# ExistentialRobotics/CORSAIR

Measured on AMD Instinct MI355X. Metric: end-to-end queries/sec (embed+retrieve+register), Scan2CAD chair, higher is better.
Workload: dtype f32 sparse conv + embedding / f64 RANSAC, k-NN, Chamfer, top-k / f16 MFMA bounds and shortlists (survivors recounted in f64)

## Files before the change

corsair_amd/csrc/ransac.h:

```cpp
#pragma once
#include "common.h"

namespace cs {

struct RansacProb {
  int64_t off;
  int32_t m;
  int32_t est_k;
  int32_t best_cnt;
  int32_t best_itr;
  unsigned long long best_err;
  int32_t done;
  int32_t iters;
  int32_t n_cand;
  int32_t chunk_max;
  double best_T[12];
};

__device__ __forceinline__ RansacProb prob_view(const RansacProb* probs, int p) {
  RansacProb v = {};
  v.off = probs[p].off;
  v.m = probs[p].m;
  v.est_k = __atomic_load_n(&probs[p].est_k, __ATOMIC_RELAXED);
  v.done = __atomic_load_n(&probs[p].done, __ATOMIC_RELAXED);
  return v;
}

constexpr int XCD_SLOTS = 64;
struct XcdTab {
  int32_t v[8 * XCD_SLOTS];
};
__device__ __forceinline__ int xcd_problem(const int32_t* __restrict__ xcd_ptr, const XcdTab& tab, int i) {
  return xcd_ptr ? xcd_ptr[i] : tab.v[i];
}

constexpr int BMAX = 16384;
constexpr int RC_CHUNK = 256;
constexpr int RC_HYP = 256;
constexpr int PF_K = 16;
constexpr int PF_PITCH = 40;
constexpr int PF_PITCH1 = 24;
__host__ __device__ constexpr int pf_pitch(int nm) { return nm == 2 ? PF_PITCH : PF_PITCH1; }
constexpr int PF_ROWS = 192;
constexpr int PF_NG = 2;
constexpr int PF_HYP = 4 * 32 * PF_NG;
constexpr int PF_STAT = 17;
constexpr float PF_SMAX = 128.0f;
constexpr int PF_S2_CAP = 1024;
constexpr double PF_TCAP = 0.75;
constexpr int FEW_MAX = 1024;

__host__ __device__ static inline int64_t pf_padded(int64_t m) { return (m + PF_ROWS - 1) / PF_ROWS * PF_ROWS; }

struct Stage2Rows {
  const _Float16* A16;
  const float* c_h;
  const unsigned* stat;
  double tcap;
  _Float16* A16s;
  float* c_hs;
  int32_t* cnt2;
};

__device__ __forceinline__ double residual2_f64(const double (&R)[12], double sx, double sy, double sz,
                                                double qx, double qy, double qz) {
  const double dx = fma(R[2], sz, fma(R[1], sy, fma(R[0], sx, R[3]))) - qx;
  const double dy = fma(R[6], sz, fma(R[5], sy, fma(R[4], sx, R[7]))) - qy;
  const double dz = fma(R[10], sz, fma(R[9], sy, fma(R[8], sx, R[11]))) - qz;
  return fma(dz, dz, fma(dy, dy, dx * dx));
}

__device__ __forceinline__ _Float16 f16_of(double v) { return (_Float16)(float)v; }

__device__ __forceinline__ void pf_centre(const double* __restrict__ sums, int p, double (&mu)[6]) {
#pragma unroll
  for (int c = 0; c < 6; ++c) mu[c] = sums[p * 6 + c];
}

__device__ __forceinline__ void pf_emit_row(const RansacProb& pr, int p, int h, int bmax, const double (&R)[3][3], double (&t)[3],
                                            const unsigned* __restrict__ stat, const double* __restrict__ sums, double thr2,
                                            double tcap, _Float16* __restrict__ A16, float* __restrict__ c_h) {
  {
    double mu[6];
    pf_centre(sums, p, mu);
#pragma unroll
    for (int a = 0; a < 3; ++a) t[a] = t[a] + (R[a][0] * mu[0] + R[a][1] * mu[1] + R[a][2] * mu[2]) - mu[3 + a];
  }
  const double smax = (double)__uint_as_float(stat[p * PF_STAT]);
  const double tt = t[0] * t[0] + t[1] * t[1] + t[2] * t[2];
  const double tn = sqrt(tt);
  double a[16];
  a[0] = 1.0;
#pragma unroll
  for (int b = 0; b < 3; ++b) a[1 + b] = 2.0 * (R[0][b] * t[0] + R[1][b] * t[1] + R[2][b] * t[2]);
#pragma unroll
  for (int x = 0; x < 3; ++x)
#pragma unroll
    for (int b = 0; b < 3; ++b) a[4 + 3 * x + b] = -2.0 * R[x][b];
#pragma unroll
  for (int x = 0; x < 3; ++x) a[13 + x] = -2.0 * t[x];
  double dev = 0.0;
#pragma unroll
  for (int x = 0; x < 3; ++x)
#pragma unroll
    for (int y = 0; y < 3; ++y) {
      const double e = R[0][x] * R[0][y] + R[1][x] * R[1][y] + R[2][x] * R[2][y] - (x == y ? 1.0 : 0.0);
      dev = fmax(dev, fabs(e));
    }
  bool usable = smax <= (double)PF_SMAX && tn <= 4.0 * (double)PF_SMAX && dev < 1.0e-3;
  if (tcap > 0.0) usable = usable && tn <= tcap * smax;
  usable = usable && thr2 < 3.0e4;
  const double beta = tcap > 0.0 ? smax * smax : 0.0;
#pragma unroll
  for (int k = 0; k < 16; ++k) usable = usable && fabs(a[k]) < 6.0e4;
  union {
    _Float16 h[PF_K];
    uint4 v[2];
  } row;
  double drop = 0.0;
#pragma unroll
  for (int k = 0; k < 16; ++k) {
    const _Float16 hi = usable ? f16_of(a[k]) : (_Float16)0.0f;
    row.h[k] = hi;
    if (usable) drop += fabs(a[k] - (double)hi) * (double)__uint_as_float(stat[p * PF_STAT + 1 + k]);
  }
  uint4* dst = reinterpret_cast<uint4*>(A16 + ((int64_t)p * bmax + h) * PF_K);
  dst[0] = row.v[0];
  dst[1] = row.v[1];
  const double w = 2.0 * smax + tn;
  const double eps = 2.5e-5 * w * w + 6.0e-6 + 3.0 * dev * smax * smax + 1.000001 * drop;
  c_h[(int64_t)p * bmax + h] = usable ? __double2float_rd((tt + beta) - (thr2 + eps)) : -1.0f;
}

struct RansacIn {
  RansacProb* probs;
  int n_prob, m_max;
  int64_t tot1;
  float* pk;
  float4* pair32;
};
struct Front {
  int it0 = 0, b = 0, par = 0;
  bool pf = false, on_side = false;
  XcdTab xtab;
  const int32_t* xcd_prob = nullptr;
  int pslots = 1;
};

void ransac_launch_pack(const RansacIn& in, const float* src, const float* tgt, hipStream_t s);
void ransac_launch_hyp(const RansacIn& in, const Front& f, int ransac_n, uint64_t seed, int force_jacobi, double* hyp,
                       const unsigned* pf_stat, const double* pf_sums, double thr2, double tcap, _Float16* A16, float* c_h,
                       int32_t* cnt_zero, hipStream_t s);
void ransac_launch_images(const RansacIn& in, const int64_t* off16, const float* src, const float* tgt, double* sums,
                          unsigned* stat, unsigned long long* chk_stats, _Float16* B32, _Float16* B16, double tcap,
                          hipStream_t s);
unsigned ransac_launch_prefilter(int nm, const RansacIn& in, const int64_t* off16, const _Float16* B, const _Float16* A16,
                                 const float* c_h, const Front& f, int tiles, int splits, int32_t* cnt_up,
                                 unsigned long long* trace, const int32_t* n_list, hipStream_t s);
void ransac_launch_survivors(const RansacIn& in, const Front& f, const int32_t* cnt_up, int32_t* res_cnt,
                             unsigned long long* err_by_h, int32_t* hlist, int32_t* n_surv, const Stage2Rows& s2, hipStream_t s);
void ransac_launch_check(const RansacIn& in, const Front& f, const int32_t* exact, const int32_t* cnt_up, const int32_t* hlist,
                         const int32_t* n_surv, const int32_t* cnt2, unsigned long long* stats, hipStream_t s);
void ransac_launch_count_chunk(const RansacIn& in, const double* hyp, int it0, int b, int hpw, int tiles, int splits,
                               double thr2, int32_t* res_cnt, hipStream_t s);
void ransac_launch_count_list(const RansacIn& in, const double* hyp, int it0, int b, double thr2, int32_t* res_cnt,
                              const int32_t* hlist, const int32_t* n_surv, hipStream_t s);
void ransac_launch_count_few(const RansacIn& in, const double* hyp, double thr2, double scale, int32_t* res_cnt,
                             unsigned long long* err_by_h, const int32_t* hlist, const int32_t* n_surv, int fslots,
                             const int32_t* cnt2, hipStream_t s);
void ransac_launch_err(const RansacIn& in, const double* hyp, const int32_t* cand, double thr2, double scale,
                       unsigned long long* cand_err, hipStream_t s);

}
```

corsair_amd/csrc/ransac.hip:

```cpp
#include <math.h>

#include <algorithm>
#include <atomic>
#include <vector>

#include "ransac.h"

namespace cs {

__device__ __forceinline__ int est_bound(int c, int m, int ransac_n, double log_1mc, int est_k0) {
  const double ratio = fmin(1.0, (double)c / (double)m);
  double pw = 1.0;
  for (int j = 0; j < ransac_n; ++j) pw = pw * ratio;
  const double den = log(1.0 - pw);
  if (den < 0.0) {
    const double est = log_1mc / den;
    if (est < (double)est_k0) return (int)ceil(est);
  }
  return est_k0;
}

__global__ __launch_bounds__(256) void k_ransac_scan1(RansacProb* probs, int n_prob,
                                                     const int32_t* __restrict__ res_cnt, int it0,
                                                     int bcount, int bmax, int ransac_n,
                                                     int max_iter, double log_1mc,
                                                     int32_t* __restrict__ cand, int* n_active,
                                                     const unsigned long long* __restrict__ err_by_h,
                                                     const double* __restrict__ hyp, int32_t* __restrict__ next_nsurv,
                                                     int* __restrict__ next_nactive) {
  extern __shared__ int32_t lcnt[];
  const int p = blockIdx.x;
  if (err_by_h && threadIdx.x == 0) {
    next_nsurv[p] = 0;
    if (p == 0) *next_nactive = 0;
  }
  RansacProb pr = probs[p];
  if (pr.done) return;
  const int seg = (bcount + 63) / 64;
  {
    const int32_t* g = res_cnt + (int64_t)p * bmax;
    for (int h = threadIdx.x; h < bcount; h += 256) lcnt[h + h / seg] = g[h];
  }
  __syncthreads();
  if (threadIdx.x >= 64) return;
  const int lane = threadIdx.x;
  const int32_t* cnt = lcnt + lane;
  const int s0 = lane * seg, s1 = min(bcount, s0 + seg);
  int lmax = 0;
  for (int h = s0; h < s1; ++h)
    if (it0 + h < pr.est_k) lmax = max(lmax, cnt[h]);
  int incl = lmax;
#pragma unroll
  for (int off = 1; off < 64; off <<= 1) {
    const int o = __shfl_up(incl, off);
    if (lane >= off) incl = max(incl, o);
  }
  int pre = __shfl_up(incl, 1);
  if (lane == 0) pre = 0;
  pre = max(pre, pr.best_cnt);
  int stop = 0x7fffffff;
  {
    int cur = pre;
    int ek = cur > pr.best_cnt ? est_bound(cur, pr.m, ransac_n, log_1mc, pr.est_k) : pr.est_k;
    for (int h = s0; h < s1; ++h) {
      if (it0 + h >= ek) {
        stop = h;
        break;
      }
      const int c = cnt[h];
      if (c > cur) {
        cur = c;
        ek = est_bound(cur, pr.m, ransac_n, log_1mc, pr.est_k);
      }
    }
  }
#pragma unroll
  for (int off = 32; off >= 1; off >>= 1) stop = min(stop, __shfl_xor(stop, off));
  if (stop > bcount) stop = bcount;
  int cmax = 0;
  for (int h = s0; h < min(s1, stop); ++h) cmax = max(cmax, cnt[h]);
#pragma unroll
  for (int off = 32; off >= 1; off >>= 1) cmax = max(cmax, __shfl_xor(cmax, off));
  int new_ek = pr.est_k;
  if (cmax > pr.best_cnt) new_ek = est_bound(cmax, pr.m, ransac_n, log_1mc, pr.est_k);
  int ncand = 0;
  unsigned long long e_min = ~0ULL;
  int h_min = 0x7fffffff;
  if (cmax > 0 && cmax >= pr.best_cnt) {
    if (err_by_h) {
      for (int h = s0; h < min(s1, stop); ++h)
        if (cnt[h] == cmax) {
          const unsigned long long e = err_by_h[(int64_t)p * bmax + h];
          if (e < e_min) {
            e_min = e;
            h_min = h;
          }
        }
#pragma unroll
      for (int off = 32; off >= 1; off >>= 1) {
        const unsigned long long eo = __shfl_xor(e_min, off);
        const int ho = __shfl_xor(h_min, off);
        if (eo < e_min || (eo == e_min && ho < h_min)) {
          e_min = eo;
          h_min = ho;
        }
      }
    } else {
      int mine = 0;
      for (int h = s0; h < min(s1, stop); ++h) mine += cnt[h] == cmax;
      int incl2 = mine;
#pragma unroll
      for (int off = 1; off < 64; off <<= 1) {
        const int o = __shfl_up(incl2, off);
        if (lane >= off) incl2 += o;
      }
      int pos = incl2 - mine;
      ncand = __shfl(incl2, 63);
      for (int h = s0; h < min(s1, stop); ++h)
        if (cnt[h] == cmax) cand[(int64_t)p * bmax + pos++] = h;
    }
  }
  if (lane == 0) {
    const int consumed = it0 + stop;
    pr.est_k = new_ek;
    pr.n_cand = ncand;
    pr.chunk_max = cmax;
    if (consumed >= pr.est_k || consumed >= max_iter) {
      pr.done = 1;
      pr.iters = consumed < max_iter ? consumed : max_iter;
    } else {
      atomicAdd(n_active, 1);
    }
    if (err_by_h && h_min != 0x7fffffff && (cmax > pr.best_cnt || e_min < pr.best_err)) {
      pr.best_cnt = cmax;
      pr.best_err = e_min;
      pr.best_itr = it0 + h_min;
      for (int c = 0; c < 12; ++c) pr.best_T[c] = hyp[((int64_t)p * 12 + c) * bmax + h_min];
    }
    probs[p] = pr;
  }
}

__global__ void k_ransac_scan2(RansacProb* probs, int n_prob, const double* __restrict__ hyp,
                               const int32_t* __restrict__ cand,
                               const unsigned long long* __restrict__ cand_err, int by_h, int it0,
                               int bmax, int32_t* __restrict__ next_nsurv, int* __restrict__ next_nactive) {
  const int p = blockIdx.x * blockDim.x + threadIdx.x;
  if (p >= n_prob) return;
  next_nsurv[p] = 0;
  if (p == 0) *next_nactive = 0;
  RansacProb pr = probs[p];
  if (pr.n_cand <= 0) return;
  bool changed = false;
  int best_h = -1;
  for (int c = 0; c < pr.n_cand; ++c) {
    const unsigned long long e = cand_err[(int64_t)p * bmax + (by_h ? cand[(int64_t)p * bmax + c] : c)];
    if (pr.chunk_max > pr.best_cnt || e < pr.best_err) {
      pr.best_cnt = pr.chunk_max;
      pr.best_err = e;
      best_h = cand[(int64_t)p * bmax + c];
      changed = true;
    }
  }
  pr.n_cand = 0;
  if (changed) {
    pr.best_itr = it0 + best_h;
    for (int c = 0; c < 12; ++c) pr.best_T[c] = hyp[((int64_t)p * 12 + c) * bmax + best_h];
  }
  probs[p] = pr;
}

__global__ void k_ransac_finish(const RansacProb* __restrict__ probs, int n_prob, double scale,
                                float* __restrict__ T, int32_t* __restrict__ inliers,
                                double* __restrict__ rmse, int32_t* __restrict__ iters) {
  const int p = blockIdx.x * blockDim.x + threadIdx.x;
  if (p >= n_prob) return;
  const RansacProb pr = probs[p];
  float* o = T + (int64_t)p * 16;
  if (pr.best_cnt > 0) {
    for (int c = 0; c < 12; ++c) o[c] = (float)pr.best_T[c];
  } else {
    for (int c = 0; c < 12; ++c) o[c] = (c % 5 == 0) ? 1.f : 0.f;
  }
  o[12] = 0.f;
  o[13] = 0.f;
  o[14] = 0.f;
  o[15] = 1.f;
  if (inliers) inliers[p] = pr.best_cnt;
  if (rmse)
    rmse[p] = pr.best_cnt > 0 ? sqrt(((double)pr.best_err / scale) / (double)pr.best_cnt) : 0.0;
  if (iters) iters[p] = pr.iters;
}

}

using namespace cs;

namespace {
std::atomic<unsigned long long> g_pf_stats[5];

struct PinnedScratch {
  char* p = nullptr;
  size_t n = 0;
  ~PinnedScratch() {
    if (p) (void)hipHostFree(p);
  }
};
thread_local PinnedScratch t_pinned;
char* pinned_scratch(size_t bytes) {
  if (t_pinned.n < bytes) {
    if (t_pinned.p) (void)hipHostFree(t_pinned.p);
    t_pinned.p = nullptr;
    t_pinned.n = 0;
    void* q = nullptr;
    if (hipHostMalloc(&q, bytes, hipHostMallocDefault) != hipSuccess) return nullptr;
    t_pinned.p = static_cast<char*>(q);
    t_pinned.n = bytes;
  }
  return t_pinned.p;
}

struct Options {
  bool prefilter;
  bool check;
  int pf_nm;
  bool stage2;
  int first_chunk;
  int force_jacobi;
  bool overlap;
  int trace_it0;
  const char* trace_file;
};
Options read_options() {
  const char* pf = getenv("CS_RANSAC_PREFILTER");
  const char* ck = getenv("CS_RANSAC_CHECK");
  const char* k = getenv("CS_RANSAC_PF_K");
  const char* s2 = getenv("CS_RANSAC_STAGE2");
  const char* first = getenv("CS_RANSAC_FIRST");
  const char* jac = getenv("CS_RANSAC_JACOBI");
  const char* ov = getenv("CS_RANSAC_OVERLAP");
  const char* tr = getenv("CS_PF_TRACE");
  const char* trf = getenv("CS_PF_TRACE_FILE");
  Options o;
  o.prefilter = !(pf && pf[0] == '0');
  o.check = ck && ck[0] == '1';
  o.pf_nm = (k && atoi(k) == 32) ? 2 : 1;
  o.stage2 = !(s2 && s2[0] == '0');
  o.first_chunk = ((std::min(std::max(first ? atoi(first) : 64, 64), BMAX) + 63) / 64) * 64;
  o.force_jacobi = jac && atoi(jac) != 0;
  o.overlap = !(ov && ov[0] == '0');
  o.trace_it0 = tr ? atoi(tr) : -1;
  o.trace_file = trf ? trf : "/tmp/pf_trace.bin";
  return o;
}

struct Scratch {
  int n_prob = 0;
  size_t st_probs = 0, st_surv = 0, st_cnt = 0, st_bytes = 0;
  PoolBuf<char> state;
  char* h_state = nullptr;
  PoolBuf<float> pk;
  PoolBuf<float4> pair32;
  PoolBuf<double> hyp;
  PoolBuf<int32_t> res_cnt, cand;
  PoolBuf<unsigned long long> cand_err;
  PoolBuf<int64_t> off16;
  PoolBuf<_Float16> B16, A16;
  PoolBuf<float> c_h;
  PoolBuf<int32_t> cnt_up, hlist;
  PoolBuf<unsigned> pf_stat;
  PoolBuf<double> pf_sums;
  PoolBuf<_Float16> B32, A16s;
  PoolBuf<float> c_hs;
  PoolBuf<int32_t> cnt2;
  PoolBuf<int32_t> exact_dbg;
  PoolBuf<unsigned long long> chk_stats;
  PoolBuf<int32_t> xcd_buf;
  PoolBuf<unsigned long long> trace;
  size_t trace_cap = 1;

  bool alloc(int n, int64_t tot1, int64_t rows16, int pf_nm, bool pf, bool stage2, bool check, bool tracing) {
    n_prob = n;
    st_probs = sizeof(RansacProb) * (size_t)n;
    st_surv = ((sizeof(int32_t) * (size_t)n + 7) / 8) * 8;
    st_cnt = st_surv + 8;
    st_bytes = st_probs + 2 * st_cnt;
    h_state = pinned_scratch(st_bytes);
    const size_t nb = (size_t)n * BMAX, ns2 = (size_t)n * PF_S2_CAP;
    if (tracing) trace_cap = (size_t)8 * n * 64 * 16 * 16;
    return h_state && state.alloc(st_bytes) && pk.alloc((size_t)tot1 * 6) && pair32.alloc((size_t)tot1 * 2) &&
           hyp.alloc(2 * nb * 12) && res_cnt.alloc(nb) && cand.alloc(nb) && cand_err.alloc(nb) && off16.alloc(n + 1) &&
           B16.alloc(pf ? (size_t)rows16 * pf_pitch(pf_nm) : 8) && A16.alloc(pf ? 2 * nb * PF_K : 8) &&
           c_h.alloc(pf ? 2 * nb : 1) && cnt_up.alloc(pf ? 2 * nb : 1) && hlist.alloc(pf ? nb : 1) &&
           pf_stat.alloc((size_t)n * PF_STAT) && pf_sums.alloc((size_t)n * 6) &&
           B32.alloc(stage2 ? (size_t)rows16 * PF_PITCH : 8) && A16s.alloc(stage2 ? ns2 * PF_K : 8) &&
           c_hs.alloc(stage2 ? ns2 : 1) && cnt2.alloc(stage2 ? ns2 : 1) &&
           exact_dbg.alloc(check ? nb : 1) && chk_stats.alloc(4) && xcd_buf.alloc((size_t)16 * n) && trace.alloc(trace_cap);
  }
  RansacProb* probs() const { return reinterpret_cast<RansacProb*>(state.p); }
  int32_t* nsurv(int par) const { return reinterpret_cast<int32_t*>(state.p + st_probs + par * st_cnt); }
  int* nactive(int par) const { return reinterpret_cast<int*>(state.p + st_probs + par * st_cnt + st_surv); }
  const int32_t* h_nsurv(int par) const { return reinterpret_cast<const int32_t*>(h_state + st_probs + par * st_cnt); }
  int h_nactive(int par) const { return *reinterpret_cast<const int*>(h_state + st_probs + par * st_cnt + st_surv); }
  double* hyp_of(int par) const { return hyp.p + (size_t)par * n_prob * 12 * BMAX; }
  _Float16* A16_of(int par) const { return A16.p + (size_t)par * n_prob * BMAX * PF_K; }
  float* c_h_of(int par) const { return c_h.p + (size_t)par * n_prob * BMAX; }
  int32_t* cnt_up_of(int par) const { return cnt_up.p + (size_t)par * n_prob * BMAX; }
  int32_t* xcd_of(int par) const { return xcd_buf.p + (size_t)par * 8 * n_prob; }
};

struct Event {
  hipEvent_t e = nullptr;
  ~Event() {
    if (e) (void)hipEventDestroy(e);
  }
};
struct SideDrain {
  hipStream_t st = nullptr;
  bool clean = false;
  ~SideDrain() {
    if (st && !clean) (void)hipStreamSynchronize(st);
  }
};

struct RansacCall {
  int n_prob = 0, ransac_n = 0, max_iter = 0, m_max = 0;
  uint64_t seed = 0;
  int64_t total = 0, tot1 = 1;
  double thr2 = 0.0, scale = 0.0, log_1mc = 0.0, tcap = 0.0;
  Options opt;
  bool pf_alloc = false, stage2 = false, check = false;
  std::vector<RansacProb> hp;
  std::vector<int64_t> h_off16;
  std::vector<int32_t> h_xcd[2];
  Scratch sc;
  Event round_done, front_done[2], hyp_done[2];
  hipStream_t s = nullptr, side = nullptr, side_hyp = nullptr;
  SideDrain side_drain, side_hyp_drain;
  int max_surv_prev = 1 << 30;
  unsigned long long tot_surv = 0, tot_eval = 0;
  size_t trace_n = 0;

  int init(const int64_t* h_off, int n, double max_corr, int rn, int iters, double confidence, uint64_t sd, hipStream_t st);
  int setup(const float* d_src, const float* d_tgt);
  int open_streams();
  RansacIn in() const { return RansacIn{sc.probs(), n_prob, m_max, tot1, sc.pk.p, sc.pair32.p}; }
  bool prefiltered(int it0) const { return pf_alloc && it0 >= opt.first_chunk; }
  int chunk_of(int it0) const {
    const int b = it0 < opt.first_chunk ? opt.first_chunk : it0 < 512 ? 512 - it0 : (it0 < BMAX ? it0 : BMAX);
    return b > max_iter - it0 ? max_iter - it0 : b;
  }
  int chunk_splits(int tiles) const {
    int splits = (int)(4096 / ((int64_t)n_prob * tiles > 0 ? (int64_t)n_prob * tiles : 1));
    if (splits < 1) splits = 1;
    if (splits > 16) splits = 16;
    while (splits > 1 && m_max / splits < 4 * RC_CHUNK) --splits;
    return splits;
  }
  int place(int it0, int par, int* live);
  Front enqueue_front(int it0, int par, hipStream_t st);
  int back_half(const Front& cur);
  int count_chunk(const Front& cur, double eval_pairs);
  int count_survivors(const Front& cur, bool* err_known);
  bool read_back(const Front& cur);
  int finish(float* d_T, int32_t* d_inliers, double* d_rmse, int32_t* d_iters);
};

int RansacCall::init(const int64_t* h_off, int n, double max_corr, int rn, int iters, double confidence, uint64_t sd,
                     hipStream_t st) {
  n_prob = n;
  ransac_n = rn;
  max_iter = iters;
  seed = sd;
  s = st;
  total = h_off[n_prob] - h_off[0];
  tot1 = total ? total : 1;
  hp.resize(n_prob);
  h_off16.assign(n_prob + 1, 0);
  for (int p = 0; p < n_prob; ++p) {
    int64_t m = h_off[p + 1] - h_off[p];
    CS_REQUIRE(m >= 0 && m < (1LL << 24), CS_ERR_INVALID,
               "cs_ransac_batch: bad segment %d (a problem holds fewer than 2^24 correspondences)", p);
    RansacProb& pr = hp[p];
    memset(&pr, 0, sizeof(pr));
    pr.off = h_off[p];
    pr.m = (int32_t)m;
    pr.est_k = max_iter;
    pr.best_itr = -1;
    pr.done = m < ransac_n ? 1 : 0;
    if (m > m_max) m_max = (int)m;
    h_off16[p + 1] = h_off16[p] + pf_padded(m);
  }
  thr2 = max_corr * max_corr;
  int ex = 0;
  (void)frexp(thr2, &ex);
  scale = ldexp(1.0, 38 - ex);
  log_1mc = log(1.0 - confidence);
  opt = read_options();
  pf_alloc = opt.prefilter && total > 0 && max_iter > opt.first_chunk;
  stage2 = pf_alloc && opt.pf_nm == 1 && opt.stage2;
  check = pf_alloc && opt.check;
  tcap = opt.pf_nm == 2 ? 0.0 : PF_TCAP;
  const bool ok = sc.alloc(n_prob, tot1, h_off16[n_prob] ? h_off16[n_prob] : 1, opt.pf_nm, pf_alloc, stage2, check,
                           opt.trace_it0 >= 0);
  CS_REQUIRE(ok, CS_ERR_HIP, "cs_ransac_batch: scratch allocation failed");
  return CS_OK;
}

int RansacCall::setup(const float* d_src, const float* d_tgt) {
  memset(sc.h_state, 0, sc.st_bytes);
  memcpy(sc.h_state, hp.data(), sc.st_probs);
  CS_HIP_CHECK(hipMemcpyAsync(sc.state.p, sc.h_state, sc.st_bytes, hipMemcpyHostToDevice, s));
  if (pf_alloc) {
    CS_HIP_CHECK(hipMemcpyAsync(sc.off16.p, h_off16.data(), sizeof(int64_t) * (n_prob + 1),
                                hipMemcpyHostToDevice, s));
    ransac_launch_images(in(), sc.off16.p, d_src, d_tgt, sc.pf_sums.p, sc.pf_stat.p, sc.chk_stats.p,
                         opt.pf_nm == 2 ? sc.B16.p : (stage2 ? sc.B32.p : nullptr), opt.pf_nm == 1 ? sc.B16.p : nullptr, tcap, s);
    CS_LAUNCH_CHECK();
  } else if (total > 0) {
    ransac_launch_pack(in(), d_src, d_tgt, s);
    CS_LAUNCH_CHECK();
  }
  if (opt.trace_it0 >= 0) CS_HIP_CHECK(hipMemsetAsync(sc.trace.p, 0, sizeof(unsigned long long) * sc.trace_cap, s));
  return CS_OK;
}

int RansacCall::open_streams() {
  for (Event* ev : {&round_done, &front_done[0], &front_done[1], &hyp_done[0], &hyp_done[1]})
    CS_HIP_CHECK(hipEventCreateWithFlags(&ev->e, hipEventDisableTiming));
  side = opt.overlap ? side_stream() : nullptr;
  side_hyp = side ? side_stream(1) : nullptr;
  side_drain.st = side;
  side_hyp_drain.st = side_hyp;
  return CS_OK;
}

int RansacCall::place(int it0, int par, int* live) {
  std::vector<int> order;
  for (int p = 0; p < n_prob; ++p)
    if (!hp[p].done && hp[p].est_k > it0) order.push_back(p);
  *live = (int)order.size();
  std::sort(order.begin(), order.end(), [&](int a, int c) { return hp[a].m > hp[c].m; });
  std::vector<std::vector<int>> lists(8);
  int64_t load[8] = {0, 0, 0, 0, 0, 0, 0, 0};
  for (int p : order) {
    int best = 0;
    for (int x = 1; x < 8; ++x)
      if (load[x] < load[best]) best = x;
    lists[best].push_back(p);
    load[best] += pf_padded(hp[p].m);
  }
  int pslots = 1;
  for (int x = 0; x < 8; ++x) pslots = std::max(pslots, (int)lists[x].size());
  std::vector<int32_t>& tab = h_xcd[par];
  tab.assign((size_t)8 * pslots, -1);
  for (int x = 0; x < 8; ++x)
    for (size_t i = 0; i < lists[x].size(); ++i) tab[(size_t)x * pslots + i] = lists[x][i];
  return pslots;
}

Front RansacCall::enqueue_front(int it0, int par, hipStream_t st) {
  Front f;
  f.it0 = it0;
  f.b = chunk_of(it0);
  f.par = par;
  f.pf = prefiltered(it0);
  f.on_side = st != s;
  const int b = f.b;
  int live = 0;
  f.pslots = place(it0, par, &live);
  const int pslots = f.pslots;
  hipStream_t sh = (f.on_side && f.pf && side_hyp) ? side_hyp : st;
  if (pslots <= XCD_SLOTS) {
    memcpy(f.xtab.v, h_xcd[par].data(), sizeof(int32_t) * 8 * pslots);
  } else {
    (void)hipMemcpyAsync(sc.xcd_of(par), h_xcd[par].data(), sizeof(int32_t) * 8 * pslots, hipMemcpyHostToDevice, sh);
    f.xcd_prob = sc.xcd_of(par);
  }
  _Float16* A16_r = f.pf ? sc.A16_of(par) : nullptr;
  float* c_h_r = f.pf ? sc.c_h_of(par) : nullptr;
  int32_t* cnt_up_r = f.pf ? sc.cnt_up_of(par) : nullptr;
  const int ptiles = (b + PF_HYP - 1) / PF_HYP;
  int psplits = (int)((8 * 1024 + (int64_t)live * ptiles - 1) / std::max<int64_t>((int64_t)live * ptiles, 1));
  if (psplits < 1) psplits = 1;
  if (psplits > 16) psplits = 16;
  while (psplits > 1 && m_max / psplits < 8 * PF_ROWS) --psplits;
  {
    ProfScope prof("ransac_hyp", sh);
    int32_t* fz = psplits > 1 ? cnt_up_r : nullptr;
    ransac_launch_hyp(in(), f, ransac_n, seed, opt.force_jacobi, sc.hyp_of(par), sc.pf_stat.p, sc.pf_sums.p, thr2, tcap, A16_r,
                      c_h_r, fz, sh);
  }
  if (f.pf) {
    if (sh != st) {
      (void)hipEventRecord(hyp_done[par].e, sh);
      (void)hipStreamWaitEvent(st, hyp_done[par].e, 0);
    }
    ProfScope prof("ransac_pre", st);
    unsigned long long* tr = (opt.trace_it0 == it0) ? sc.trace.p : nullptr;
    const unsigned nblk = ransac_launch_prefilter(opt.pf_nm, in(), sc.off16.p, sc.B16.p, A16_r, c_h_r, f, ptiles, psplits,
                                                  cnt_up_r, tr, nullptr, st);
    if (tr) trace_n = (size_t)nblk * 16;
  }
  if (f.on_side) (void)hipEventRecord(front_done[par].e, st);
  return f;
}

int RansacCall::count_chunk(const Front& cur, double eval_pairs) {
  const int b = cur.b;
  const int hpw = b <= 64 ? 64 : RC_HYP;
  const int tiles = (b + hpw - 1) / hpw;
  const int splits = chunk_splits(tiles);
  if (splits > 1 || hpw != RC_HYP)
    CS_HIP_CHECK(hipMemset2DAsync(sc.res_cnt.p, sizeof(int32_t) * BMAX, 0, sizeof(int32_t) * b, n_prob, s));
  ProfScope prof("ransac_eval", s, 30.0 * eval_pairs);
  ransac_launch_count_chunk(in(), sc.hyp_of(cur.par), cur.it0, b, hpw, tiles, splits, thr2, sc.res_cnt.p, s);
  return CS_OK;
}

int RansacCall::count_survivors(const Front& cur, bool* err_known) {
  const int b = cur.b;
  const double* hyp_r = sc.hyp_of(cur.par);
  const int32_t* cnt_up_r = sc.cnt_up_of(cur.par);
  int32_t* const d_nsurv = sc.nsurv(cur.par);
  const int surv_cap = std::min(max_surv_prev, b);
  const bool few = max_surv_prev <= FEW_MAX || b <= FEW_MAX;
  const bool run_s2 = stage2 && few && surv_cap <= PF_S2_CAP;
  Stage2Rows s2rows{};
  if (run_s2) {
    s2rows.A16 = sc.A16_of(cur.par);
    s2rows.c_h = sc.c_h_of(cur.par);
    s2rows.stat = sc.pf_stat.p;
    s2rows.tcap = tcap;
    s2rows.A16s = sc.A16s.p;
    s2rows.c_hs = sc.c_hs.p;
    s2rows.cnt2 = sc.cnt2.p;
  }
  ransac_launch_survivors(in(), cur, cnt_up_r, sc.res_cnt.p, sc.cand_err.p, sc.hlist.p, d_nsurv, s2rows, s);
  {
    ProfScope prof("ransac_eval", s);
    if (few) {
      if (run_s2) {
        const int s2tiles = std::max(1, (std::min(b, PF_S2_CAP) + PF_HYP - 1) / PF_HYP);
        int s2splits = 8;
        while (s2splits > 1 && m_max / s2splits < 8 * PF_ROWS) --s2splits;
        ransac_launch_prefilter(2, in(), sc.off16.p, sc.B32.p, sc.A16s.p, sc.c_hs.p, cur, s2tiles, s2splits, sc.cnt2.p, nullptr,
                                d_nsurv, s);
      }
      const int fslots = surv_cap <= 256 ? 4 : 8;
      ransac_launch_count_few(in(), hyp_r, thr2, scale, sc.res_cnt.p, sc.cand_err.p, sc.hlist.p, d_nsurv, fslots,
                              run_s2 ? sc.cnt2.p : nullptr, s);
      *err_known = true;
    } else {
      ransac_launch_count_list(in(), hyp_r, cur.it0, b, thr2, sc.res_cnt.p, sc.hlist.p, d_nsurv, s);
    }
  }
  if (check) {
    const int tiles = (b + RC_HYP - 1) / RC_HYP;
    const int splits = chunk_splits(tiles);
    CS_HIP_CHECK(hipMemset2DAsync(sc.exact_dbg.p, sizeof(int32_t) * BMAX, 0, sizeof(int32_t) * b, n_prob, s));
    ransac_launch_count_chunk(in(), hyp_r, cur.it0, b, RC_HYP, tiles, splits, thr2, sc.exact_dbg.p, s);
    ransac_launch_check(in(), cur, sc.exact_dbg.p, cnt_up_r, sc.hlist.p, d_nsurv, run_s2 ? sc.cnt2.p : nullptr, sc.chk_stats.p, s);
  }
  return CS_OK;
}

int RansacCall::back_half(const Front& cur) {
  const int it0 = cur.it0, b = cur.b;
  double eval_pairs = 0.0;
  for (int p = 0; p < n_prob; ++p) {
    if (hp[p].done) continue;
    const int nh = std::min(hp[p].est_k - it0, b);
    if (nh > 0) {
      eval_pairs += (double)nh * (double)hp[p].m;
      tot_eval += (unsigned long long)nh;
    }
  }
  bool err_known = false;
  if (!cur.pf) {
    if (int rc = count_chunk(cur, eval_pairs)) return rc;
  } else {
    prof_add_units("ransac_pre", 30.0 * eval_pairs);
    if (int rc = count_survivors(cur, &err_known)) return rc;
  }
  static const hipError_t scan1_lds = hipFuncSetAttribute(
      reinterpret_cast<const void*>(k_ransac_scan1), hipFuncAttributeMaxDynamicSharedMemorySize, 80 * 1024);
  CS_REQUIRE(scan1_lds == hipSuccess, CS_ERR_HIP, "cs_ransac_batch: cannot reserve LDS for k_ransac_scan1");
  RansacProb* const d_probs = sc.probs();
  const double* hyp_r = sc.hyp_of(cur.par);
  int32_t* const next_nsurv = sc.nsurv(cur.par ^ 1);
  int* const next_nactive = sc.nactive(cur.par ^ 1);
  hipLaunchKernelGGL(k_ransac_scan1, dim3((unsigned)n_prob), dim3(256), sizeof(int32_t) * (b + 64), s, d_probs, n_prob,
                     sc.res_cnt.p, it0, b, BMAX, ransac_n, max_iter, log_1mc, sc.cand.p, sc.nactive(cur.par),
                     err_known ? sc.cand_err.p : (const unsigned long long*)nullptr, hyp_r, next_nsurv, next_nactive);
  if (!err_known) {
    ransac_launch_err(in(), hyp_r, sc.cand.p, thr2, scale, sc.cand_err.p, s);
    hipLaunchKernelGGL(k_ransac_scan2, dim3((unsigned)ceil_div(n_prob, 64)), dim3(64), 0, s,
                       d_probs, n_prob, hyp_r, sc.cand.p, sc.cand_err.p, 0, it0, BMAX, next_nsurv, next_nactive);
  }
  CS_LAUNCH_CHECK();
  return CS_OK;
}

bool RansacCall::read_back(const Front& cur) {
  if (cur.pf) {
    const int32_t* h_surv = sc.h_nsurv(cur.par);
    max_surv_prev = 0;
    for (int p = 0; p < n_prob; ++p)
      if (!hp[p].done) {
        tot_surv += (unsigned long long)h_surv[p];
        if (h_surv[p] > max_surv_prev) max_surv_prev = h_surv[p];
      }
  }
  memcpy(hp.data(), sc.h_state, sc.st_probs);
  return sc.h_nactive(cur.par) != 0;
}

int RansacCall::finish(float* d_T, int32_t* d_inliers, double* d_rmse, int32_t* d_iters) {
  if (trace_n) {
    std::vector<unsigned long long> ht(trace_n);
    CS_HIP_CHECK(hipMemcpy(ht.data(), sc.trace.p, sizeof(unsigned long long) * trace_n, hipMemcpyDeviceToHost));
    FILE* f = fopen(opt.trace_file, "wb");
    if (f) {
      fwrite(ht.data(), sizeof(unsigned long long), trace_n, f);
      fclose(f);
    }
  }
  g_pf_stats[3] += tot_surv;
  g_pf_stats[4] += tot_eval;
  if (check) {
    unsigned long long h_stats[4] = {0, 0, 0, 0};
    CS_HIP_CHECK(hipMemcpyAsync(h_stats, sc.chk_stats.p, sizeof(h_stats), hipMemcpyDeviceToHost, s));
    CS_HIP_CHECK(hipStreamSynchronize(s));
    g_pf_stats[0] += h_stats[0];
    g_pf_stats[1] += h_stats[1];
    g_pf_stats[2] += h_stats[2];
    CS_REQUIRE(h_stats[0] == 0, CS_ERR_INTERNAL,
               "cs_ransac_batch: prefilter bound violated for %llu hypotheses", h_stats[0]);
  }
  hipLaunchKernelGGL(k_ransac_finish, dim3((unsigned)ceil_div(n_prob, 64)), dim3(64), 0, s,
                     sc.probs(), n_prob, scale, d_T, d_inliers, d_rmse, d_iters);
  CS_LAUNCH_CHECK();
  CS_HIP_CHECK(hipStreamSynchronize(s));
  side_drain.clean = true;
  side_hyp_drain.clean = true;
  return CS_OK;
}
}

extern "C" {

void cs_ransac_prefilter_stats(uint64_t out[5], int reset) {
  for (int i = 0; i < 5; ++i) {
    if (out) out[i] = g_pf_stats[i].load();
    if (reset) g_pf_stats[i].store(0);
  }
}

int cs_ransac_batch(const float* d_src, const float* d_tgt, const int64_t* h_off, int n_prob,
                    double max_corr, int ransac_n, int max_iter, double confidence, uint64_t seed,
                    float* d_T, int32_t* d_inliers, double* d_rmse, int32_t* d_iters,
                    void* stream) {
  CS_REQUIRE(h_off && d_T, CS_ERR_INVALID, "cs_ransac_batch: NULL argument");
  CS_REQUIRE(ransac_n >= 3 && ransac_n <= 64, CS_ERR_INVALID,
             "cs_ransac_batch: ransac_n %d not in [3, 64]", ransac_n);
  CS_REQUIRE(max_corr > 0.0 && max_iter >= 1, CS_ERR_INVALID,
             "cs_ransac_batch: need max_corr > 0 and max_iter >= 1");
  CS_REQUIRE(confidence > 0.0 && confidence <= 1.0, CS_ERR_INVALID,
             "cs_ransac_batch: confidence must be in (0, 1]");
  if (n_prob <= 0) return CS_OK;
  hipStream_t s = (hipStream_t)stream;
  pool_use_stream(s);
  const int64_t total = h_off[n_prob] - h_off[0];
  CS_REQUIRE(h_off[0] == 0 && total >= 0, CS_ERR_INVALID, "cs_ransac_batch: bad offsets");
  CS_REQUIRE(total == 0 || (d_src && d_tgt), CS_ERR_INVALID, "cs_ransac_batch: NULL correspondences");
  RansacCall c;
  if (int rc = c.init(h_off, n_prob, max_corr, ransac_n, max_iter, confidence, seed, s)) return rc;
  if (int rc = c.setup(d_src, d_tgt)) return rc;
  if (int rc = c.open_streams()) return rc;

  Front cur = c.enqueue_front(0, 0, s);
  CS_LAUNCH_CHECK();
  bool side_pending = false;
  int side_par = 0;
  while (true) {
    if (cur.on_side) {
      CS_HIP_CHECK(hipStreamWaitEvent(s, c.front_done[cur.par].e, 0));
      side_pending = false;
    }
    if (int rc = c.back_half(cur)) return rc;
    CS_HIP_CHECK(hipMemcpyAsync(c.sc.h_state, c.sc.state.p, c.sc.st_bytes, hipMemcpyDeviceToHost, s));
    CS_HIP_CHECK(hipEventRecord(c.round_done.e, s));
    Front nxt;
    const int it1 = cur.it0 + cur.b;
    const bool have_next = it1 < max_iter;
    if (have_next) {
      nxt = c.enqueue_front(it1, cur.par ^ 1, (c.side && cur.pf && c.prefiltered(it1)) ? c.side : s);
      if (nxt.on_side) {
        side_pending = true;
        side_par = nxt.par;
      }
      CS_LAUNCH_CHECK();
    }
    CS_HIP_CHECK(hipEventSynchronize(c.round_done.e));
    const bool active = c.read_back(cur);
    if (!active || !have_next) break;
    cur = nxt;
  }
  if (side_pending) CS_HIP_CHECK(hipStreamWaitEvent(s, c.front_done[side_par].e, 0));
  return c.finish(d_T, d_inliers, d_rmse, d_iters);
}

}
```

corsair_amd/csrc/ransac_hyp.hip:

```cpp
#include "ransac.h"
#include "exact_div.h"
#include "horn.h"

namespace cs {


__global__ void k_ransac_pack(const float* __restrict__ src, const float* __restrict__ tgt,
                              int64_t n, float* __restrict__ pk, float4* __restrict__ pair32) {
  int64_t i = blockIdx.x * (int64_t)blockDim.x + threadIdx.x;
  if (i >= n) return;
  pair32[2 * i + 0] = make_float4(src[3 * i + 0], src[3 * i + 1], src[3 * i + 2], tgt[3 * i + 0]);
  pair32[2 * i + 1] = make_float4(tgt[3 * i + 1], tgt[3 * i + 2], 0.f, 0.f);
  pk[0 * n + i] = src[3 * i + 0];
  pk[1 * n + i] = src[3 * i + 1];
  pk[2 * n + i] = src[3 * i + 2];
  pk[3 * n + i] = tgt[3 * i + 0];
  pk[4 * n + i] = tgt[3 * i + 1];
  pk[5 * n + i] = tgt[3 * i + 2];
}

__device__ __forceinline__ void centroid_div(double (&cs_)[3], double (&ct_)[3], double dn, double inv_n) {
  bool fast = inv_n != 0.0;
#pragma unroll
  for (int a = 0; a < 3; ++a) fast = fast && exact_div_ok(cs_[a]) && exact_div_ok(ct_[a]);
  if (fast) {
#pragma unroll
    for (int a = 0; a < 3; ++a) {
      cs_[a] = exact_div(cs_[a], dn, inv_n);
      ct_[a] = exact_div(ct_[a], dn, inv_n);
    }
  } else {
#pragma unroll
    for (int a = 0; a < 3; ++a) {
      cs_[a] = cs_[a] / dn;
      ct_[a] = ct_[a] / dn;
    }
  }
}

template <int RN>
__attribute__((amdgpu_waves_per_eu(5, 5)))
__global__ __launch_bounds__(256) void k_ransac_hyp(const RansacProb* probs,
                                                    const float4* __restrict__ pair32, int it0,
                                                    int bcount, int bmax, int ransac_n, double inv_n,
                                                    uint64_t seed,
                                                    const int32_t* __restrict__ xcd_prob, const XcdTab xcd_tab,
                                                    int slots, int tiles, int force_jacobi,
                                                    double* __restrict__ hyp,
                                                    const unsigned* __restrict__ pf_stat, const double* __restrict__ pf_sums,
                                                    double thr2, double tcap, _Float16* __restrict__ A16,
                                                    float* __restrict__ c_h, int32_t* __restrict__ cnt_zero) {
  const int xcd = blockIdx.x & 7;
  const int item = blockIdx.x >> 3;
  const int slot = item / tiles;
  const int p = xcd_problem(xcd_prob, xcd_tab, xcd * slots + slot);
  if (p < 0) return;
  const int h = (item - slot * tiles) * blockDim.x + threadIdx.x;
  if (h >= bcount) return;
  if (cnt_zero) cnt_zero[(int64_t)p * bmax + h] = 0;
  const RansacProb pr = prob_view(probs, p);
  const int itr = it0 + h;
  if (pr.done || itr >= pr.est_k) return;
  const uint32_t m = (uint32_t)pr.m;
  double cs_[3] = {0, 0, 0}, ct_[3] = {0, 0, 0};
  double S[3][3] = {{0, 0, 0}, {0, 0, 0}, {0, 0, 0}};
  if (RN > 0) {
    float pa[RN > 0 ? RN : 1][6];
#pragma unroll
    for (int j = 0; j < RN; ++j) {
      const int64_t i = pr.off + rng_index(seed, (uint64_t)itr, (uint64_t)j, m);
      const float4 a = pair32[2 * i], b = pair32[2 * i + 1];
      pa[j][0] = a.x; pa[j][1] = a.y; pa[j][2] = a.z; pa[j][3] = a.w; pa[j][4] = b.x; pa[j][5] = b.y;
#pragma unroll
      for (int c = 0; c < 3; ++c) {
        cs_[c] += (double)pa[j][c];
        ct_[c] += (double)pa[j][3 + c];
      }
    }
    centroid_div(cs_, ct_, (double)RN, inv_n);
#pragma unroll
    for (int j = 0; j < RN; ++j) {
#pragma unroll
      for (int c = 0; c < 6; ++c) asm volatile("" : "+v"(pa[j][c]));
      const double ds[3] = {(double)pa[j][0] - cs_[0], (double)pa[j][1] - cs_[1], (double)pa[j][2] - cs_[2]};
      const double dt[3] = {(double)pa[j][3] - ct_[0], (double)pa[j][4] - ct_[1], (double)pa[j][5] - ct_[2]};
#pragma unroll
      for (int x = 0; x < 3; ++x)
#pragma unroll
        for (int y = 0; y < 3; ++y) S[x][y] = fma(ds[x], dt[y], S[x][y]);
    }
  } else {
    for (int j = 0; j < ransac_n; ++j) {
      const int64_t i = pr.off + rng_index(seed, (uint64_t)itr, (uint64_t)j, m);
      const float4 a = pair32[2 * i], b = pair32[2 * i + 1];
      cs_[0] += (double)a.x;
      cs_[1] += (double)a.y;
      cs_[2] += (double)a.z;
      ct_[0] += (double)a.w;
      ct_[1] += (double)b.x;
      ct_[2] += (double)b.y;
    }
    centroid_div(cs_, ct_, (double)ransac_n, inv_n);
    for (int j = 0; j < ransac_n; ++j) {
      const int64_t i = pr.off + rng_index(seed, (uint64_t)itr, (uint64_t)j, m);
      const float4 a = pair32[2 * i], b = pair32[2 * i + 1];
      const double ds[3] = {(double)a.x - cs_[0], (double)a.y - cs_[1], (double)a.z - cs_[2]};
      const double dt[3] = {(double)a.w - ct_[0], (double)b.x - ct_[1], (double)b.y - ct_[2]};
#pragma unroll
      for (int a = 0; a < 3; ++a)
#pragma unroll
        for (int b = 0; b < 3; ++b) S[a][b] = fma(ds[a], dt[b], S[a][b]);
    }
  }
  double N[4][4], V[4][4];
  N[0][0] = S[0][0] + S[1][1] + S[2][2];
  N[0][1] = S[1][2] - S[2][1];
  N[0][2] = S[2][0] - S[0][2];
  N[0][3] = S[0][1] - S[1][0];
  N[1][1] = S[0][0] - S[1][1] - S[2][2];
  N[1][2] = S[0][1] + S[1][0];
  N[1][3] = S[2][0] + S[0][2];
  N[2][2] = -S[0][0] + S[1][1] - S[2][2];
  N[2][3] = S[1][2] + S[2][1];
  N[3][3] = -S[0][0] - S[1][1] + S[2][2];
  N[1][0] = N[0][1];
  N[2][0] = N[0][2];
  N[3][0] = N[0][3];
  N[2][1] = N[1][2];
  N[3][1] = N[1][3];
  N[3][2] = N[2][3];
  double qv[4];
  if (force_jacobi || !horn_qcp(S, N, qv)) {
    jacobi4(N, V);
    double best = N[0][0];
    qv[0] = V[0][0]; qv[1] = V[1][0]; qv[2] = V[2][0]; qv[3] = V[3][0];
#pragma unroll
    for (int c = 1; c < 4; ++c) {
      if (N[c][c] > best) {
        best = N[c][c];
        qv[0] = V[0][c];
        qv[1] = V[1][c];
        qv[2] = V[2][c];
        qv[3] = V[3][c];
      }
    }
  }
  double qw = qv[0], qx = qv[1], qy = qv[2], qz = qv[3];
  const double qn = sqrt(qw * qw + qx * qx + qy * qy + qz * qz);
  qw = qw / qn;
  qx = qx / qn;
  qy = qy / qn;
  qz = qz / qn;
  double R[3][3];
  R[0][0] = 1.0 - 2.0 * (qy * qy + qz * qz);
  R[0][1] = 2.0 * (qx * qy - qw * qz);
  R[0][2] = 2.0 * (qx * qz + qw * qy);
  R[1][0] = 2.0 * (qx * qy + qw * qz);
  R[1][1] = 1.0 - 2.0 * (qx * qx + qz * qz);
  R[1][2] = 2.0 * (qy * qz - qw * qx);
  R[2][0] = 2.0 * (qx * qz - qw * qy);
  R[2][1] = 2.0 * (qy * qz + qw * qx);
  R[2][2] = 1.0 - 2.0 * (qx * qx + qy * qy);
  double* o = hyp + ((int64_t)p * 12) * bmax + h;
  double tv[3];
#pragma unroll
  for (int a = 0; a < 3; ++a) {
    const double t = ct_[a] - (R[a][0] * cs_[0] + R[a][1] * cs_[1] + R[a][2] * cs_[2]);
    tv[a] = t;
    o[(int64_t)(4 * a + 0) * bmax] = R[a][0];
    o[(int64_t)(4 * a + 1) * bmax] = R[a][1];
    o[(int64_t)(4 * a + 2) * bmax] = R[a][2];
    o[(int64_t)(4 * a + 3) * bmax] = t;
  }
  if (A16) pf_emit_row(pr, p, h, bmax, R, tv, pf_stat, pf_sums, thr2, tcap, A16, c_h);
}

void ransac_launch_pack(const RansacIn& in, const float* src, const float* tgt, hipStream_t s) {
  hipLaunchKernelGGL(k_ransac_pack, dim3((unsigned)ceil_div(in.tot1, 256)), dim3(256), 0, s, src, tgt, in.tot1, in.pk,
                     in.pair32);
}

void ransac_launch_hyp(const RansacIn& in, const Front& f, int ransac_n, uint64_t seed, int force_jacobi, double* hyp,
                       const unsigned* pf_stat, const double* pf_sums, double thr2, double tcap, _Float16* A16, float* c_h,
                       int32_t* cnt_zero, hipStream_t s) {
  const int htiles = (f.b + 255) / 256;
  const auto kernel = ransac_n == 10 ? k_ransac_hyp<10> : k_ransac_hyp<0>;
  hipLaunchKernelGGL(kernel, dim3((unsigned)(8 * f.pslots * htiles)), dim3(256), 0, s, in.probs, in.pair32, f.it0, f.b, BMAX,
                     ransac_n, exact_div_recip((double)ransac_n), seed, f.xcd_prob, f.xtab, f.pslots, htiles, force_jacobi, hyp,
                     pf_stat, pf_sums, thr2, tcap, A16, c_h, cnt_zero);
}
}
```

Measured before the change: 2046.

## Skip f64 hypothesis stores in prefilter pass; recompute only survivors later

The hypothesis kernel no longer writes the full f64 rotation/translation matrices for every hypothesis when the f16 prefilter is active (unless the check mode or a bypass problem requires it). A new list-driven launch recomputes the Horn solve and stores f64 hypotheses only for the prefilter survivors before exact counting. This trades store bandwidth over the whole batch for a second, smaller recompute pass plus an extra kernel launch.

```diff
diff --git a/corsair_amd/csrc/ransac.h b/corsair_amd/csrc/ransac.h
--- a/corsair_amd/csrc/ransac.h
+++ b/corsair_amd/csrc/ransac.h
@@ -150,7 +150,9 @@
 void ransac_launch_pack(const RansacIn& in, const float* src, const float* tgt, hipStream_t s);
 void ransac_launch_hyp(const RansacIn& in, const Front& f, int ransac_n, uint64_t seed, int force_jacobi, double* hyp,
                        const unsigned* pf_stat, const double* pf_sums, double thr2, double tcap, _Float16* A16, float* c_h,
-                       int32_t* cnt_zero, hipStream_t s);
+                       int32_t* cnt_zero, bool keep_rec, hipStream_t s);
+void ransac_launch_hyp_list(const RansacIn& in, const Front& f, int ransac_n, uint64_t seed, int force_jacobi, double* hyp,
+                            const unsigned* pf_stat, const int32_t* hlist, const int32_t* n_surv, int list_cap, hipStream_t s);
 void ransac_launch_images(const RansacIn& in, const int64_t* off16, const float* src, const float* tgt, double* sums,
                           unsigned* stat, unsigned long long* chk_stats, _Float16* B32, _Float16* B16, double tcap,
                           hipStream_t s);
diff --git a/corsair_amd/csrc/ransac.hip b/corsair_amd/csrc/ransac.hip
--- a/corsair_amd/csrc/ransac.hip
+++ b/corsair_amd/csrc/ransac.hip
@@ -489,7 +489,7 @@
     ProfScope prof("ransac_hyp", sh);
     int32_t* fz = psplits > 1 ? cnt_up_r : nullptr;
     ransac_launch_hyp(in(), f, ransac_n, seed, opt.force_jacobi, sc.hyp_of(par), sc.pf_stat.p, sc.pf_sums.p, thr2, tcap, A16_r,
-                      c_h_r, fz, sh);
+                      c_h_r, fz, check, sh);
   }
   if (f.pf) {
     if (sh != st) {
@@ -539,6 +539,8 @@
   ransac_launch_survivors(in(), cur, cnt_up_r, sc.res_cnt.p, sc.cand_err.p, sc.hlist.p, d_nsurv, s2rows, s);
   {
     ProfScope prof("ransac_eval", s);
+    ransac_launch_hyp_list(in(), cur, ransac_n, seed, opt.force_jacobi, sc.hyp_of(cur.par), sc.pf_stat.p, sc.hlist.p, d_nsurv,
+                           b, s);
     if (few) {
       if (run_s2) {
         const int s2tiles = std::max(1, (std::min(b, PF_S2_CAP) + PF_HYP - 1) / PF_HYP);
diff --git a/corsair_amd/csrc/ransac_hyp.hip b/corsair_amd/csrc/ransac_hyp.hip
--- a/corsair_amd/csrc/ransac_hyp.hip
+++ b/corsair_amd/csrc/ransac_hyp.hip
@@ -1,3 +1,5 @@
+#include <algorithm>
+
 #include "ransac.h"
 #include "exact_div.h"
 #include "horn.h"
@@ -49,14 +51,20 @@
                                                     double* __restrict__ hyp,
                                                     const unsigned* __restrict__ pf_stat, const double* __restrict__ pf_sums,
                                                     double thr2, double tcap, _Float16* __restrict__ A16,
-                                                    float* __restrict__ c_h, int32_t* __restrict__ cnt_zero) {
+                                                    float* __restrict__ c_h, int32_t* __restrict__ cnt_zero,
+                                                    const int32_t* __restrict__ hlist, const int32_t* __restrict__ n_surv,
+                                                    int keep_rec) {
   const int xcd = blockIdx.x & 7;
   const int item = blockIdx.x >> 3;
   const int slot = item / tiles;
   const int p = xcd_problem(xcd_prob, xcd_tab, xcd * slots + slot);
   if (p < 0) return;
-  const int h = (item - slot * tiles) * blockDim.x + threadIdx.x;
-  if (h >= bcount) return;
+  const int e = (item - slot * tiles) * blockDim.x + threadIdx.x;
+  if (e >= (hlist ? min(n_surv[p], bcount) : bcount)) return;
+  const bool bypass = (A16 || hlist) && !(__uint_as_float(pf_stat[p * PF_STAT]) <= PF_SMAX);
+  if (hlist && bypass) return;
+  const bool record = !A16 || keep_rec || bypass;
+  const int h = hlist ? hlist[(int64_t)p * bmax + e] : e;
   if (cnt_zero) cnt_zero[(int64_t)p * bmax + h] = 0;
   const RansacProb pr = prob_view(probs, p);
   const int itr = it0 + h;
@@ -167,10 +175,12 @@
   for (int a = 0; a < 3; ++a) {
     const double t = ct_[a] - (R[a][0] * cs_[0] + R[a][1] * cs_[1] + R[a][2] * cs_[2]);
     tv[a] = t;
-    o[(int64_t)(4 * a + 0) * bmax] = R[a][0];
-    o[(int64_t)(4 * a + 1) * bmax] = R[a][1];
-    o[(int64_t)(4 * a + 2) * bmax] = R[a][2];
-    o[(int64_t)(4 * a + 3) * bmax] = t;
+    if (record) {
+      o[(int64_t)(4 * a + 0) * bmax] = R[a][0];
+      o[(int64_t)(4 * a + 1) * bmax] = R[a][1];
+      o[(int64_t)(4 * a + 2) * bmax] = R[a][2];
+      o[(int64_t)(4 * a + 3) * bmax] = t;
+    }
   }
   if (A16) pf_emit_row(pr, p, h, bmax, R, tv, pf_stat, pf_sums, thr2, tcap, A16, c_h);
 }
@@ -182,11 +192,22 @@
 
 void ransac_launch_hyp(const RansacIn& in, const Front& f, int ransac_n, uint64_t seed, int force_jacobi, double* hyp,
                        const unsigned* pf_stat, const double* pf_sums, double thr2, double tcap, _Float16* A16, float* c_h,
-                       int32_t* cnt_zero, hipStream_t s) {
+                       int32_t* cnt_zero, bool keep_rec, hipStream_t s) {
   const int htiles = (f.b + 255) / 256;
   const auto kernel = ransac_n == 10 ? k_ransac_hyp<10> : k_ransac_hyp<0>;
   hipLaunchKernelGGL(kernel, dim3((unsigned)(8 * f.pslots * htiles)), dim3(256), 0, s, in.probs, in.pair32, f.it0, f.b, BMAX,
                      ransac_n, exact_div_recip((double)ransac_n), seed, f.xcd_prob, f.xtab, f.pslots, htiles, force_jacobi, hyp,
-                     pf_stat, pf_sums, thr2, tcap, A16, c_h, cnt_zero);
-}
-}
+                     pf_stat, pf_sums, thr2, tcap, A16, c_h, cnt_zero, (const int32_t*)nullptr, (const int32_t*)nullptr,
+                     keep_rec ? 1 : 0);
+}
+
+void ransac_launch_hyp_list(const RansacIn& in, const Front& f, int ransac_n, uint64_t seed, int force_jacobi, double* hyp,
+                            const unsigned* pf_stat, const int32_t* hlist, const int32_t* n_surv, int list_cap, hipStream_t s) {
+  const int ltiles = std::max(1, (std::min(list_cap, f.b) + 255) / 256);
+  const auto kernel = ransac_n == 10 ? k_ransac_hyp<10> : k_ransac_hyp<0>;
+  hipLaunchKernelGGL(kernel, dim3((unsigned)(8 * f.pslots * ltiles)), dim3(256), 0, s, in.probs, in.pair32, f.it0, f.b, BMAX,
+                     ransac_n, exact_div_recip((double)ransac_n), seed, f.xcd_prob, f.xtab, f.pslots, ltiles, force_jacobi, hyp,
+                     pf_stat, (const double*)nullptr, 0.0, 0.0, (_Float16*)nullptr, (float*)nullptr, (int32_t*)nullptr, hlist,
+                     n_surv, 1);
+}
+}
```

Result: no change. 2055, median of 2 (+0.5%).
